# amisr/volumetricinterp

Measured on AMD Instinct MI355X. Metric: fit+eval timesteps/sec, higher is better.
Workload: dtype f64

## Files before the change

volumetricinterp_amd/csrc/vi_fit.hip:

```cpp
#include "vi_common.h"
#include "vi_solver.h"
#include "vi_gemm_device.h"

#include <rocsolver/rocsolver.h>

#include <cstdlib>

namespace {

inline unsigned nblk(int64_t n, int b) { return (unsigned)((n + b - 1) / b); }

__global__ void k_scale_rows(int64_t P, int N, const double* __restrict__ At, const double* __restrict__ W,
                             double* __restrict__ B, int tvalid)
{
    const int64_t p = (int64_t)blockIdx.x * blockDim.x + threadIdx.x;
    const int n = blockIdx.y, t = blockIdx.z;
    if (p >= P) return;
    const int ts = t < tvalid ? t : tvalid - 1;
    B[((int64_t)t * N + n) * P + p] = At[(int64_t)n * P + p] * W[(int64_t)ts * P + p];
}

__global__ void k_mul(int64_t n, const double* __restrict__ a, const double* __restrict__ b, double* __restrict__ o)
{
    const int64_t i = (int64_t)blockIdx.x * blockDim.x + threadIdx.x;
// ... 674 lines not shown
                                             tmp, N, s, d_H, N, s, &zero, d_dC, N, s, (rocblas_int)T));
    return VI_OK;
}

extern "C" int vi_eigvals_f64(vi_ctx* c, int64_t B, int32_t N, double* d_X, double* d_lam, int32_t* d_sweeps)
{
    VI_REQUIRE(c && d_X && d_lam, "null argument");
    VI_REQUIRE(B >= 0 && N > 0, "bad size");
    if (B == 0) return VI_OK;
    if (!vi_jacobi_supported(N)) {
        vi_set_error("vi_eigvals_f64: N=%d outside the in-LDS Jacobi range", N);
        return VI_ERR_UNSUPPORTED;
    }
    VI_HIP(hipSetDevice(c->device));
    const bool qr = qr_enabled(N);
    const size_t hhb = qr ? up16(vi_qr_hh_bytes(N)) : 0;
    cold_dst d{};
    d.cap = cold_max_sweeps(N);
    double* yz;
    int rc = ws_carve(c, [&](ws_carver& w) {
        d.log = w.take<char>((size_t)B * vi_jacobi_log_bytes(N, d.cap));
        d.scl = w.take<double>(B);
        yz = w.take<double>((size_t)B * N);
        d.C = w.take<double>((size_t)B * N);
        if (qr) {
            d.y1 = w.take<double>((size_t)B * N);
            d.hh = w.take<double>((size_t)B * (hhb / 8));
            d.scr = w.take<double>((size_t)B * N * N);
        }
    });
    if (rc != VI_OK) return rc;
    d.hh_stride = (int64_t)hhb;
    d.sweeps = d_sweeps;
    d.lam = d_lam;
    VI_HIP(hipMemsetAsync(yz, 0, (size_t)B * N * sizeof(double), c->stream));
    return cold_solve(c, B, N, d_X, yz, nullptr, 2.220446049250313e-16, d);
}

namespace {
size_t log_record_bytes(int N)
{
    return vi_jacobi_log_bytes(N, JACOBI_MAX_SWEEPS) + (qr_enabled(N) ? up16(vi_qr_hh_bytes(N)) : 0);
}

struct prep_ws {
    double *scl, *lam, *y1;
    double *T0, *T1;
    double *scrT, *scrD;
    const double** parr;
    int64_t np;
    void decompose(ws_carver& w, int64_t n, int N)
    {
        scl = w.take<double>(n);
        lam = w.take<double>((size_t)n * N);
        y1 = w.take<double>((size_t)n * N);
    }
    void matrices(ws_carver& w, int64_t n, int N)
    {
        T0 = w.take<double>((size_t)n * N * N);
        T1 = w.take<double>((size_t)n * N * N);
    }
    void finish(ws_carver& w, int64_t n, int N)
    {
        scrT = w.take<double>((size_t)GEMM_GROUP * N * N);
        scrD = w.take<double>((size_t)GEMM_GROUP * N * N);
        np = group_pad(n);
        parr = w.take<const double*>((size_t)6 * np);
    }
};

int prep_decompose(vi_ctx* c, int64_t bc, int N, const double* d_AWA, const int32_t* recc, const double* alpha0c,
                   const double* d_R, const double* d_y, double rcond, double* Cc, int32_t* rankc, void* log, int* nrd,
                   const prep_ws& p)
{
    hipLaunchKernelGGL(k_form_system, dim3((unsigned)bc), dim3(256), 0, c->stream, N * N, d_AWA, recc, alpha0c, d_R, p.T0);
    cold_dst d{};
    d.C = Cc;
    d.rank = rankc;
    d.C_back = true;
    d.log = log;
    d.hh = (double*)((char*)log + vi_jacobi_log_bytes(N, JACOBI_MAX_SWEEPS));
    d.log_stride = d.hh_stride = (int64_t)log_record_bytes(N);
    d.scl = p.scl;
    d.y1 = p.y1;
    d.scr = p.T1;
    d.lam = p.lam;
    d.lam_raw = 1;
    d.nround = nrd;
    d.cap = JACOBI_MAX_SWEEPS;
    return cold_solve(c, bc, N, p.T0, d_y, recc, rcond, d);
}

int prep_finish(vi_ctx* c, int64_t bc, int N, const void* log, const int* nrd, const double* d_AWA, const int32_t* recc,
                const double* d_R, const double* d_y, double* Vc, double* D1c, double* D2c, double* ytc, const prep_ws& p)
{
    const int NN = N * N;
    double *T0 = p.T0, *T1 = p.T1, *scrT = p.scrT, *scrD = p.scrD;
    const double** pT0 = p.parr;
    const double** pV = pT0 + p.np;
    const double** pT1 = pV + p.np;
    const double** pR = pT1 + p.np;
    const double** pD1 = pR + p.np;
    const double** pD2 = pD1 + p.np;
    const size_t recb = log_record_bytes(N);
    int rc = vi_jacobi_vectors(c, bc, N, log, JACOBI_MAX_SWEEPS, nrd, Vc, (int64_t)(recb / 16));
    if (rc != VI_OK) return rc;
    if (qr_enabled(N)) {
        const double* hh = (const double*)((const char*)log + vi_jacobi_log_bytes(N, JACOBI_MAX_SWEEPS));
        if ((rc = vi_qr_back_mat(c, bc, N, hh, Vc, (int64_t)(recb / 8))) != VI_OK) return rc;
    }
    hipLaunchKernelGGL(k_form_system, dim3((unsigned)bc), dim3(256), 0, c->stream, NN, d_AWA, recc, nullptr, nullptr, T0);
    VI_HIP(hipGetLastError());
    if ((rc = group_ptrs(c, bc, T0, NN, nullptr, 0, pT0)) != VI_OK) return rc;
    if ((rc = group_ptrs(c, bc, Vc, NN, nullptr, 0, pV)) != VI_OK) return rc;
    if ((rc = group_ptrs(c, bc, T1, NN, scrT, NN, pT1)) != VI_OK) return rc;
    if ((rc = group_ptrs(c, bc, d_R, 0, nullptr, 0, pR)) != VI_OK) return rc;
    if ((rc = group_ptrs(c, bc, D1c, NN, scrD, NN, pD1)) != VI_OK) return rc;
    if ((rc = group_ptrs(c, bc, D2c, NN, scrD, NN, pD2)) != VI_OK) return rc;
    if ((rc = gemm_groups(c, rocblas_operation_none, rocblas_operation_none, N, N, N, pT0, N, pV, N, pT1, N, bc)) != VI_OK) return rc;
    if ((rc = gemm_groups(c, rocblas_operation_transpose, rocblas_operation_none, N, N, N, pV, N, pT1, N, pD1, N, bc)) != VI_OK)
        return rc;
    if ((rc = gemm_groups(c, rocblas_operation_none, rocblas_operation_none, N, N, N, pR, N, pV, N, pT1, N, bc)) != VI_OK) return rc;
    if ((rc = gemm_groups(c, rocblas_operation_transpose, rocblas_operation_none, N, N, N, pV, N, pT1, N, pD2, N, bc)) != VI_OK)
        return rc;
    hipLaunchKernelGGL(k_vt_vec, dim3((unsigned)bc), dim3(256), 0, c->stream, N, Vc, nullptr, d_y, recc, ytc);
    VI_HIP(hipGetLastError());
    return VI_OK;
}
}

extern "C" int vi_warm_prepare_f64(vi_ctx* c, int64_t B, int32_t N, const double* d_AWA, const int32_t* d_rec,
                                   const double* d_alpha0, const double* d_R, const double* d_y, double rcond,
                                   double* d_C, int32_t* d_rank, double* d_V, double* d_D1, double* d_D2, double* d_yt)
{
    VI_REQUIRE(c && d_AWA && d_rec && d_alpha0 && d_R && d_y && d_C && d_V && d_D1 && d_D2 && d_yt, "null argument");
    VI_REQUIRE(B >= 0 && N > 0, "bad size");
    if (B == 0) return VI_OK;
    if (!vi_jacobi_vectors_supported(N)) {
        vi_set_error("vi_warm_prepare_f64: N=%d outside the in-LDS Jacobi range", N);
        return VI_ERR_UNSUPPORTED;
    }
    VI_HIP(hipSetDevice(c->device));
    const int NN = N * N;
    const size_t recb = log_record_bytes(N);
    const size_t per = recb + (size_t)(2 * N + 1) * sizeof(double) + sizeof(int) + (size_t)2 * NN * sizeof(double) + 6 * sizeof(void*);
    const int64_t Bc = chunk_size((size_t)4 << 30, per, B);
    void* log;
    int* nrd;
    prep_ws p{};
    int rc = ws_carve(c, [&](ws_carver& w) {
        log = w.take<char>((size_t)Bc * recb);
        p.decompose(w, Bc, N);
        p.matrices(w, Bc, N);
        p.finish(w, Bc, N);
        nrd = w.take<int>(Bc);
    });
    if (rc != VI_OK) return rc;
    return for_chunks(B, Bc, [&](int64_t i0, int64_t bc) -> int {
        const int r = prep_decompose(c, bc, N, d_AWA, d_rec + i0, d_alpha0 + i0, d_R, d_y, rcond, d_C + i0 * N,
                                     d_rank ? d_rank + i0 : nullptr, log, nrd, p);
        if (r != VI_OK) return r;
        return prep_finish(c, bc, N, log, nrd, d_AWA, d_rec + i0, d_R, d_y, d_V + i0 * NN, d_D1 + i0 * NN, d_D2 + i0 * NN,
                           d_yt + i0 * N, p);
    });
}

extern "C" size_t vi_rotation_log_bytes(int32_t N) { return log_record_bytes(N); }
extern "C" int vi_max_sweeps(void) { return JACOBI_MAX_SWEEPS; }
extern "C" int vi_cold_max_sweeps(int32_t N) { return cold_max_sweeps(N); }
double vi_floor_warm() { return JACOBI_FLOOR_WARM; }

namespace {
double walk_tolerance()
{
    static const double v = vi_env_double("VINTERP_WALK_TOL", 1e-6);
    return v;
}
}

extern "C" int vi_decompose_f64(vi_ctx* c, int64_t B, int32_t N, const double* d_AWA, const int32_t* d_rec,
                                const double* d_alpha0, const double* d_R, const double* d_y, double rcond, double* d_C,
                                int32_t* d_rank, void* d_log, int32_t* d_nround)
{
    VI_REQUIRE(c && d_AWA && d_rec && d_alpha0 && d_R && d_y && d_C && d_log && d_nround, "null argument");
    VI_REQUIRE(B >= 0 && N > 0, "bad size");
    if (B == 0) return VI_OK;
    if (!vi_jacobi_vectors_supported(N)) {
        vi_set_error("vi_decompose_f64: N=%d outside the in-LDS Jacobi range", N);
        return VI_ERR_UNSUPPORTED;
    }
    VI_HIP(hipSetDevice(c->device));
    prep_ws p{};
    int rc = ws_carve(c, [&](ws_carver& w) {
        p.decompose(w, B, N);
        p.matrices(w, B, N);
    });
    if (rc != VI_OK) return rc;
    return prep_decompose(c, B, N, d_AWA, d_rec, d_alpha0, d_R, d_y, rcond, d_C, d_rank, d_log, d_nround, p);
}

extern "C" int vi_warm_finish_f64(vi_ctx* c, int64_t B, int32_t N, const void* d_log, const int32_t* d_nround,
                                  const double* d_AWA, const int32_t* d_rec, const double* d_R, const double* d_y,
                                  double* d_V, double* d_D1, double* d_D2, double* d_yt)
{
    VI_REQUIRE(c && d_log && d_nround && d_AWA && d_rec && d_R && d_y && d_V && d_D1 && d_D2 && d_yt, "null argument");
    VI_REQUIRE(B >= 0 && N > 0, "bad size");
    if (B == 0) return VI_OK;
    if (!vi_jacobi_vectors_supported(N)) {
        vi_set_error("vi_warm_finish_f64: N=%d outside the in-LDS Jacobi range", N);
        return VI_ERR_UNSUPPORTED;
    }
    VI_HIP(hipSetDevice(c->device));
    prep_ws p{};
    int rc = ws_carve(c, [&](ws_carver& w) {
        p.matrices(w, B, N);
        p.finish(w, B, N);
    });
    if (rc != VI_OK) return rc;
    return prep_finish(c, B, N, d_log, d_nround, d_AWA, d_rec, d_R, d_y, d_V, d_D1, d_D2, d_yt, p);
}

extern "C" int vi_warm_solve_f64(vi_ctx* c, int64_t B, int32_t N, const double* d_D1, const double* d_D2,
                                 const double* d_yt, const double* d_V, const int32_t* d_slot, const double* d_alpha,
                                 double rcond, double* d_C, int32_t* d_rank, int32_t* d_sweeps)
{
    VI_REQUIRE(c && d_D1 && d_D2 && d_yt && d_V && d_slot && d_alpha && d_C, "null argument");
    VI_REQUIRE(B >= 0 && N > 0, "bad size");
    if (B == 0) return VI_OK;
    if (!vi_jacobi_supported(N)) {
        vi_set_error("vi_warm_solve_f64: N=%d outside the in-LDS Jacobi range", N);
        return VI_ERR_UNSUPPORTED;
    }
    VI_HIP(hipSetDevice(c->device));
    const int NN = N * N;
    const size_t logb = vi_jacobi_log_bytes(N, JACOBI_MAX_SWEEPS);
    const int64_t Bc = chunk_size((size_t)4 << 30, logb, B);
    void* log;
    double *scl, *X, *cp;
    int rc = ws_carve(c, [&](ws_carver& w) {
        log = w.take<char>((size_t)Bc * logb);
        scl = w.take<double>(Bc);
        X = w.take<double>((size_t)Bc * NN);
        cp = w.take<double>((size_t)Bc * N);
    });
    if (rc != VI_OK) return rc;
    return for_chunks(B, Bc, [&](int64_t i0, int64_t bc) -> int {
        form_pair_scaled(c, bc, NN, d_D1, d_D2, d_slot + i0, d_slot + i0, d_alpha + i0, X, scl);
        VI_HIP(hipGetLastError());
        const int r = vi_jacobi_solve(c, bc, N, X, scl, d_yt, d_slot + i0, rcond, cp, d_rank ? d_rank + i0 : nullptr, log,
                                      JACOBI_MAX_SWEEPS, d_sweeps ? d_sweeps + i0 : nullptr, nullptr, 0, nullptr, JACOBI_FLOOR_WARM);
        if (r != VI_OK) return r;
        hipLaunchKernelGGL(k_v_vec, dim3((unsigned)bc), dim3(256), (size_t)N * sizeof(double), c->stream, N, d_V,
                           d_slot + i0, cp, d_C + i0 * N);
        VI_HIP(hipGetLastError());
        return VI_OK;
    });
}

namespace {
template <int BS>
__global__ __launch_bounds__(BS) void k_reg_floor(int NN, const double* __restrict__ AWA, const double* __restrict__ R,
                                                  double* __restrict__ out)
{
    __shared__ double red[BS / 64];
    const double* Xt = AWA + (int64_t)blockIdx.x * NN;
    double mn = 1.7976931348623157e308;
    for (int e = threadIdx.x; e < NN; e += BS) {
        const double r = fabs(R[e]);
        if (r > 0.0) mn = fmin(mn, (0.25 * 2.220446049250313e-16) * fabs(Xt[e]) / r);
    }
    for (int o = 32; o > 0; o >>= 1) mn = fmin(mn, __shfl_xor(mn, o));
    if ((threadIdx.x & 63) == 0) red[threadIdx.x >> 6] = mn;
    __syncthreads();
    if (threadIdx.x == 0) {
        for (int q = 1; q < BS / 64; ++q) mn = fmin(mn, red[q]);
        out[blockIdx.x] = mn;
    }
}
}

extern "C" int vi_reg_floor_f64(vi_ctx* c, int64_t T, int32_t N, const double* d_AWA, const double* d_R, double* d_out)
{
    VI_REQUIRE(c && d_AWA && d_R && d_out, "null argument");
    VI_REQUIRE(T >= 0 && N > 0, "bad size");
    if (T == 0) return VI_OK;
    VI_HIP(hipSetDevice(c->device));
    hipLaunchKernelGGL(k_reg_floor<256>, dim3((unsigned)T), dim3(256), 0, c->stream, N * N, d_AWA, d_R, d_out);
    VI_HIP(hipGetLastError());
    return VI_OK;
}

namespace {
__global__ void k_basis_ptrs(int64_t B, int NN, const double* AWA, const int* __restrict__ rec, const double* V,
                             const int* __restrict__ basis, double* T1, double* D1, const double** pA, const double** pV,
                             double** pT, double** pD)
{
    const int64_t i = (int64_t)blockIdx.x * blockDim.x + threadIdx.x;
    if (i >= B) return;
    pA[i] = AWA + (int64_t)rec[i] * NN;
    pV[i] = V + (int64_t)basis[i] * NN;
    pT[i] = T1 + i * NN;
    pD[i] = D1 + i * NN;
}
}

extern "C" int vi_basis_solve_f64(vi_ctx* c, int64_t B, int32_t N, const double* d_AWA, const double* d_y,
                                  const int32_t* d_rec, const int32_t* d_basis, const double* d_alpha, const double* d_V,
                                  const double* d_D2, double rcond, double* d_C, int32_t* d_rank, int32_t* d_sweeps)
{
    VI_REQUIRE(c && d_AWA && d_y && d_rec && d_basis && d_alpha && d_V && d_D2 && d_C, "null argument");
    VI_REQUIRE(B >= 0 && N > 0, "bad size");
    if (B == 0) return VI_OK;
    if (!vi_jacobi_supported(N)) {
        vi_set_error("vi_basis_solve_f64: N=%d outside the in-LDS Jacobi range", N);
        return VI_ERR_UNSUPPORTED;
    }
    VI_HIP(hipSetDevice(c->device));
    const int NN = N * N;
    const size_t logb = vi_jacobi_log_bytes(N, JACOBI_MAX_SWEEPS);
    const size_t per = logb + sizeof(double) + (size_t)2 * NN * sizeof(double) + (size_t)2 * N * sizeof(double) + 4 * sizeof(void*);
    const int64_t Bc = chunk_size((size_t)8 << 30, per, B, 256);
    void* log;
    double *scl, *T1, *D1, *yt, *cp;
    const double **pA, **pV;
    double **pT, **pD;
    int rc = ws_carve(c, [&](ws_carver& w) {
        log = w.take<char>((size_t)Bc * logb);
        scl = w.take<double>(Bc);
        T1 = w.take<double>((size_t)Bc * NN);
        D1 = w.take<double>((size_t)Bc * NN);
        yt = w.take<double>((size_t)Bc * N);
        cp = w.take<double>((size_t)Bc * N);
        pA = w.take<const double*>(Bc);
        pV = w.take<const double*>(Bc);
        pT = w.take<double*>(Bc);
        pD = w.take<double*>(Bc);
    });
    if (rc != VI_OK) return rc;
    const double one = 1.0, zero = 0.0;
    return for_chunks(B, Bc, [&](int64_t i0, int64_t bc) -> int {
        hipLaunchKernelGGL(k_basis_ptrs, dim3((unsigned)((bc + 255) / 256)), dim3(256), 0, c->stream, bc, NN, d_AWA,
                           d_rec + i0, d_V, d_basis + i0, T1, D1, pA, pV, pT, pD);
        VI_HIP(hipGetLastError());
        VI_ROCBLAS(rocblas_dgemm_batched(c->blas, rocblas_operation_none, rocblas_operation_none, N, N, N, &one, pA, N,
                                         pV, N, &zero, pT, N, (rocblas_int)bc));
        VI_ROCBLAS(rocblas_dgemm_batched(c->blas, rocblas_operation_transpose, rocblas_operation_none, N, N, N, &one, pV, N,
                                         (const double* const*)pT, N, &zero, pD, N, (rocblas_int)bc));
        hipLaunchKernelGGL(k_vt_vec, dim3((unsigned)bc), dim3(256), 0, c->stream, N, d_V, d_basis + i0, d_y, d_rec + i0, yt);
        form_pair_scaled(c, bc, NN, D1, d_D2, nullptr, d_basis + i0, d_alpha + i0, D1, scl);
        VI_HIP(hipGetLastError());
        const int r = vi_jacobi_solve(c, bc, N, D1, scl, yt, nullptr, rcond, cp, d_rank ? d_rank + i0 : nullptr, log,
                                      JACOBI_MAX_SWEEPS, d_sweeps ? d_sweeps + i0 : nullptr, nullptr, 0, nullptr,
                                      JACOBI_FLOOR_WARM, 0, walk_tolerance());
        if (r != VI_OK) return r;
        hipLaunchKernelGGL(k_v_vec, dim3((unsigned)bc), dim3(256), (size_t)N * sizeof(double), c->stream, N, d_V,
                           d_basis + i0, cp, d_C + i0 * N);
        VI_HIP(hipGetLastError());
        return VI_OK;
    });
}

extern "C" int vi_warm_rebase_f64(vi_ctx* c, int64_t B, int64_t nplain, int32_t N, const double* d_AWA, const double* d_R,
                                  const double* d_y, const int32_t* d_rec, const int32_t* d_slot, const double* d_alpha,
                                  double rcond, double* d_V, double* d_D1, double* d_D2, double* d_yt, double* d_C,
                                  int32_t* d_rank, int32_t* d_sweeps)
{
    VI_REQUIRE(c && d_AWA && d_R && d_y && d_rec && d_slot && d_alpha && d_V && d_D1 && d_D2 && d_yt && d_C, "null argument");
    VI_REQUIRE(B >= 0 && N > 0 && nplain >= 0 && nplain <= B, "bad size");
    if (B == 0) return VI_OK;
    if (nplain == B) return vi_warm_solve_f64(c, B, N, d_D1, d_D2, d_yt, d_V, d_slot, d_alpha, rcond, d_C, d_rank, d_sweeps);
    if (!vi_jacobi_vectors_supported(N)) {
        vi_set_error("vi_warm_rebase_f64: N=%d outside the in-LDS Jacobi range", N);
        return VI_ERR_UNSUPPORTED;
    }
    VI_HIP(hipSetDevice(c->device));
    const int NN = N * N;
    const size_t logb = vi_jacobi_log_bytes(N, JACOBI_MAX_SWEEPS);
    const size_t per = logb + sizeof(double) + sizeof(int) + (size_t)3 * NN * sizeof(double) + (size_t)N * sizeof(double) +
                       8 * sizeof(void*);
    const int64_t Bc = chunk_size((size_t)4 << 30, per, B);
    if (nplain > 0 && B > Bc) {
        int rc0 = vi_warm_solve_f64(c, nplain, N, d_D1, d_D2, d_yt, d_V, d_slot, d_alpha, rcond, d_C, d_rank, d_sweeps);
        if (rc0 != VI_OK) return rc0;
        return vi_warm_rebase_f64(c, B - nplain, 0, N, d_AWA, d_R, d_y, d_rec + nplain, d_slot + nplain, d_alpha + nplain, rcond,
                                  d_V, d_D1, d_D2, d_yt, d_C + nplain * N, d_rank ? d_rank + nplain : nullptr,
                                  d_sweeps ? d_sweeps + nplain : nullptr);
    }
    const int64_t Bcp = group_pad(Bc);
    char* log;
    double *scl, *X, *Vw, *Vn, *cp, *scrA, *scrB;
    const double **pX, **pVold, **pVw, **pVn, **pR, **pD1, **pD2;
    int* nrd;
    int rc = ws_carve(c, [&](ws_carver& w) {
        log = w.take<char>((size_t)Bc * logb);
        scl = w.take<double>(Bc);
        X = w.take<double>((size_t)Bc * NN);
        Vw = w.take<double>((size_t)Bc * NN);
        Vn = w.take<double>((size_t)Bc * NN);
        cp = w.take<double>((size_t)Bc * N);
        scrA = w.take<double>((size_t)GEMM_GROUP * NN);
        scrB = w.take<double>((size_t)GEMM_GROUP * NN);
        for (auto* pp : {&pX, &pVold, &pVw, &pVn, &pR, &pD1, &pD2}) *pp = w.take<const double*>(Bcp);
        nrd = w.take<int>(Bc);
    });
    if (rc != VI_OK) return rc;
    return for_chunks(B, Bc, [&](int64_t i0, int64_t bc) -> int {
        const int32_t* slotc = d_slot + i0;
        const int32_t* recc = d_rec + i0;
        form_pair_scaled(c, bc, NN, d_D1, d_D2, slotc, slotc, d_alpha + i0, X, scl);
        VI_HIP(hipGetLastError());
        int rc = vi_jacobi_solve(c, bc, N, X, scl, d_yt, slotc, rcond, cp, d_rank ? d_rank + i0 : nullptr, log, JACOBI_MAX_SWEEPS,
                                 d_sweeps ? d_sweeps + i0 : nullptr, nullptr, 0, nrd, JACOBI_FLOOR_WARM);
        if (rc != VI_OK) return rc;
        hipLaunchKernelGGL(k_v_vec, dim3((unsigned)bc), dim3(256), (size_t)N * sizeof(double), c->stream, N, d_V, slotc, cp,
                           d_C + i0 * N);
        VI_HIP(hipGetLastError());
        const int64_t skip = i0 == 0 ? nplain : 0;
        rc = vi_jacobi_vectors(c, bc - skip, N, log + (size_t)skip * logb, JACOBI_MAX_SWEEPS, nrd + skip, Vw);
        if (rc != VI_OK) return rc;
        slotc += skip;
        recc += skip;
        bc -= skip;
        if ((rc = group_ptrs(c, bc, d_V, NN, nullptr, 0, pVold, slotc)) != VI_OK) return rc;
        if ((rc = group_ptrs(c, bc, Vw, NN, scrA, NN, pVw)) != VI_OK) return rc;
        if ((rc = group_ptrs(c, bc, Vn, NN, scrB, NN, pVn)) != VI_OK) return rc;
        if ((rc = wg_gemm_batched(c, false, N, pVold, pVw, pVn, bc)) != VI_OK) return rc;
        hipLaunchKernelGGL(k_scatter_mat, dim3((unsigned)bc), dim3(256), 0, c->stream, NN, Vn, slotc, d_V);
        hipLaunchKernelGGL(k_form_system, dim3((unsigned)bc), dim3(256), 0, c->stream, NN, d_AWA, recc, nullptr, nullptr, X);
        VI_HIP(hipGetLastError());
        if ((rc = group_ptrs(c, bc, X, NN, nullptr, 0, pX)) != VI_OK) return rc;
        if ((rc = group_ptrs(c, bc, d_R, 0, nullptr, 0, pR)) != VI_OK) return rc;
        if ((rc = group_ptrs(c, bc, d_D1, NN, scrB, NN, pD1, slotc)) != VI_OK) return rc;
        if ((rc = group_ptrs(c, bc, d_D2, NN, scrB, NN, pD2, slotc)) != VI_OK) return rc;
        if ((rc = wg_gemm_batched(c, false, N, pX, pVn, pVw, bc)) != VI_OK) return rc;
        if ((rc = wg_gemm_batched(c, true, N, pVn, pVw, pD1, bc)) != VI_OK) return rc;
        if ((rc = wg_gemm_batched(c, false, N, pR, pVn, pVw, bc)) != VI_OK) return rc;
        if ((rc = wg_gemm_batched(c, true, N, pVn, pVw, pD2, bc)) != VI_OK) return rc;
        hipLaunchKernelGGL(k_vt_vec_slot, dim3((unsigned)bc), dim3(256), 0, c->stream, N, Vn, d_y, recc, slotc, d_yt);
        VI_HIP(hipGetLastError());
        return VI_OK;
    });
}

namespace {
__global__ void k_set_one(double* scratch, double alpha, int slot, int rec)
{
    scratch[0] = alpha;
    int* iv = reinterpret_cast<int*>(scratch + 2);
    iv[0] = slot;
    iv[1] = rec;
}
}

extern "C" int vi_warm_chi2_one_f64(vi_ctx* c, int32_t N, int64_t P, const double* d_D1, const double* d_D2,
                                    const double* d_yt, const double* d_V, int32_t slot, double alpha, double rcond,
                                    const double* d_At, int32_t rec, const double* d_W, const double* d_b,
                                    double* d_scratch, double* h_chi2)
{
    VI_REQUIRE(c && d_D1 && d_D2 && d_yt && d_V && d_At && d_W && d_b && d_scratch && h_chi2, "null argument");
    VI_REQUIRE(N > 0 && P > 0 && slot >= 0 && rec >= 0, "bad size");
    VI_HIP(hipSetDevice(c->device));
    double* d_alpha = d_scratch;
    double* d_chi = d_scratch + 1;
    int32_t* d_slot = reinterpret_cast<int32_t*>(d_scratch + 2);
    int32_t* d_rec = d_slot + 1;
    int32_t* d_sw = reinterpret_cast<int32_t*>(d_scratch + 3);
    double* d_C = d_scratch + 8;
    hipLaunchKernelGGL(k_set_one, dim3(1), dim3(1), 0, c->stream, d_scratch, alpha, (int)slot, (int)rec);
    VI_HIP(hipGetLastError());
    int rc = vi_warm_solve_f64(c, 1, N, d_D1, d_D2, d_yt, d_V, d_slot, d_alpha, rcond, d_C, nullptr, d_sw);
    if (rc != VI_OK) return rc;
    rc = vi_chi2_f64(c, 1, P, N, d_At, d_C, d_rec, d_W, d_b, d_chi);
    if (rc != VI_OK) return rc;
    VI_HIP(hipMemcpyAsync(h_chi2, d_chi, 3 * sizeof(double), hipMemcpyDeviceToHost, c->stream));
    VI_HIP(hipStreamSynchronize(c->stream));
    return VI_OK;
}

extern "C" int vi_gcv_terms_f64(vi_ctx* c, int64_t np, int64_t P, int32_t N, const double* d_At, const int32_t* d_pidx,
                                const double* d_AWA, const double* d_y, const double* d_W, const double* d_b,
                                double alpha, const double* d_R, double rcond, double* d_res)
{
    VI_REQUIRE(c && d_At && d_pidx && d_AWA && d_y && d_W && d_b && d_res, "null argument");
    VI_REQUIRE(np >= 0 && P > 0 && N > 0, "bad size");
    if (np == 0) return VI_OK;
    VI_HIP(hipSetDevice(c->device));
    const int NN = N * N;
    const int64_t Bc = chunk_size((size_t)1 << 30, (size_t)NN * sizeof(double), np);
    double* buf = nullptr;
    VI_HIP(hipMalloc((void**)&buf, (size_t)Bc * (NN + 2 * (size_t)N) * sizeof(double)));
    double* X = buf;
    double* yl = X + (size_t)Bc * NN;
    double* Cl = yl + (size_t)Bc * N;
    const int rc = for_chunks(np, Bc, [&](int64_t i0, int64_t bc) -> int {
        hipLaunchKernelGGL(k_form_loo, dim3((unsigned)bc), dim3(256), (size_t)N * sizeof(double), c->stream, N, P, d_At,
                           d_pidx + i0, d_AWA, d_y, d_W, d_b, alpha, d_R, X, yl);
        if (hipGetLastError() != hipSuccess) { vi_set_error("k_form_loo launch failed"); return VI_ERR_HIP; }
        const int r = vi_solve_trunc_f64(c, bc, N, X, yl, nullptr, rcond, Cl, nullptr, 0.0, nullptr);
        if (r != VI_OK) return r;
        hipLaunchKernelGGL(k_loo_resid, dim3((unsigned)((bc + 3) / 4)), dim3(256), 0, c->stream, bc, N, P, d_At, d_pidx + i0,
                           Cl, d_W, d_b, d_res + i0);
        if (hipGetLastError() != hipSuccess) { vi_set_error("k_loo_resid launch failed"); return VI_ERR_HIP; }
        return VI_OK;
    });
    (void)hipStreamSynchronize(c->stream);
    (void)hipFree(buf);
    return rc;
}
```

volumetricinterp_amd/csrc/vi_solver.h:

```cpp
#pragma once
#include "vi_common.h"

size_t vi_jacobi_lds_bytes(int N);
size_t vi_jacobi_log_bytes(int N, int max_sweeps);
bool vi_jacobi_supported(int N);
bool vi_jacobi_use_v2(int N);
int vi_jacobi_solve(vi_ctx* c, int64_t B, int N, const double* d_X, const double* d_scl, const double* d_y,
                    const int* d_rec, double rcond, double* d_C, int* d_rank, void* d_log, int max_sweeps,
                    int* d_sweeps, double* d_lam, int lam_raw, int* d_nround, double abs_floor, int64_t log_stride = 0,
                    double conv_tol = 0.0);
bool vi_jacobi_vectors_supported(int N);
int vi_jacobi_vectors(vi_ctx* c, int64_t B, int N, const void* d_log, int max_sweeps, const int* d_nround, double* d_V,
                      int64_t log_stride = 0);

bool vi_qr_supported(int N);
size_t vi_qr_hh_bytes(int N);
int vi_qr_precond(vi_ctx* c, int64_t B, int N, const double* d_X, const double* d_y, const int* d_rec, double* d_X1,
                  double* d_y1, double* d_hh, double* d_scr, int64_t hh_stride = 0);
int vi_qr_back_vec(vi_ctx* c, int64_t B, int N, const double* d_hh, double* d_C, int64_t hh_stride = 0);
int vi_qr_back_mat(vi_ctx* c, int64_t B, int N, const double* d_hh, double* d_V, int64_t hh_stride = 0);

double vi_floor_warm();

int vi_eval_sph_mfma(vi_model* m, int64_t Q, const double* lat, const double* lon, const double* alt, int64_t T,
                     const double* Cp, const unsigned char* hull, int F, double* out, int64_t* done);
int vi_eval_sph_split(vi_model* m, int64_t Q, const double* lat, const double* lon, const double* alt, int64_t T,
                      const double* Cp, const unsigned char* hull, int F, double* out, int* handled);
int vi_eval_resident_mfma(vi_ctx* c, int N, int64_t Q, int64_t T, const double* d_Y, const double* d_C, double* d_out, int* handled);
int vi_eval_resident_err_mfma(vi_ctx* c, int N, int64_t Q, int64_t T, const double* d_Y, const double* d_dC, double* d_out,
                              int* handled);
```

Measured before the change: 3365.

## Fuse basis rotation V^T A V, projection and scaling into one MFMA kernel

Replaces the two batched rocBLAS DGEMMs, the pointer-setup kernel, the V^T y kernel and the pair-scaling pass in the basis solve with one per-item kernel. The new kernel computes V^T·A·V with f64 MFMA, keeps V and A in registers or LDS, writes only the lower-triangular blocks, adds alpha·D2, and applies a power-of-two scale. This removes several launches and the global round trip of the intermediate T1 matrix, and halves the workspace per item, which allows larger chunks. The old BLAS path stays available through an environment variable. The risks are that each block handles one matrix, which may leave the GPU underused for small N, and that the non-resident path for large N reloads V from global memory.

After: 3435, median of 6. +2.1%, better.

```diff
diff --git a/volumetricinterp_amd/csrc/vi_fit.hip b/volumetricinterp_amd/csrc/vi_fit.hip
--- a/volumetricinterp_amd/csrc/vi_fit.hip
+++ b/volumetricinterp_amd/csrc/vi_fit.hip
@@ -1000,6 +1000,17 @@
     pT[i] = T1 + i * NN;
     pD[i] = D1 + i * NN;
 }
+
+bool walk_form_blas()
+{
+    static const bool v = vi_env_is("VINTERP_WALK_FORM", "blas");
+    return v;
+}
+int walk_chunk_cap()
+{
+    static const int v = vi_env_int("VINTERP_WALK_CHUNK", 0);
+    return v;
+}
 }
 
 extern "C" int vi_basis_solve_f64(vi_ctx* c, int64_t B, int32_t N, const double* d_AWA, const double* d_y,
@@ -1015,39 +1026,49 @@
     }
     VI_HIP(hipSetDevice(c->device));
     const int NN = N * N;
+    const bool blas = walk_form_blas();
     const size_t logb = vi_jacobi_log_bytes(N, JACOBI_MAX_SWEEPS);
-    const size_t per = logb + sizeof(double) + (size_t)2 * NN * sizeof(double) + (size_t)2 * N * sizeof(double) + 4 * sizeof(void*);
-    const int64_t Bc = chunk_size((size_t)8 << 30, per, B, 256);
+    size_t per = logb + sizeof(double) + (size_t)NN * sizeof(double) + (size_t)2 * N * sizeof(double);
+    if (blas) per += (size_t)NN * sizeof(double) + 4 * sizeof(void*);
+    int64_t Bc = chunk_size((size_t)8 << 30, per, B, 256);
+    if (walk_chunk_cap() > 0 && Bc > walk_chunk_cap()) Bc = walk_chunk_cap();
     void* log;
-    double *scl, *T1, *D1, *yt, *cp;
-    const double **pA, **pV;
-    double **pT, **pD;
+    double *scl, *T1 = nullptr, *X, *yt, *cp;
+    const double **pA = nullptr, **pV = nullptr;
+    double **pT = nullptr, **pD = nullptr;
     int rc = ws_carve(c, [&](ws_carver& w) {
         log = w.take<char>((size_t)Bc * logb);
         scl = w.take<double>(Bc);
-        T1 = w.take<double>((size_t)Bc * NN);
-        D1 = w.take<double>((size_t)Bc * NN);
+        X = w.take<double>((size_t)Bc * NN);
         yt = w.take<double>((size_t)Bc * N);
         cp = w.take<double>((size_t)Bc * N);
-        pA = w.take<const double*>(Bc);
-        pV = w.take<const double*>(Bc);
-        pT = w.take<double*>(Bc);
-        pD = w.take<double*>(Bc);
+        if (blas) {
+            T1 = w.take<double>((size_t)Bc * NN);
+            pA = w.take<const double*>(Bc);
+            pV = w.take<const double*>(Bc);
+            pT = w.take<double*>(Bc);
+            pD = w.take<double*>(Bc);
+        }
     });
     if (rc != VI_OK) return rc;
     const double one = 1.0, zero = 0.0;
     return for_chunks(B, Bc, [&](int64_t i0, int64_t bc) -> int {
-        hipLaunchKernelGGL(k_basis_ptrs, dim3((unsigned)((bc + 255) / 256)), dim3(256), 0, c->stream, bc, NN, d_AWA,
-                           d_rec + i0, d_V, d_basis + i0, T1, D1, pA, pV, pT, pD);
-        VI_HIP(hipGetLastError());
-        VI_ROCBLAS(rocblas_dgemm_batched(c->blas, rocblas_operation_none, rocblas_operation_none, N, N, N, &one, pA, N,
-                                         pV, N, &zero, pT, N, (rocblas_int)bc));
-        VI_ROCBLAS(rocblas_dgemm_batched(c->blas, rocblas_operation_transpose, rocblas_operation_none, N, N, N, &one, pV, N,
-                                         (const double* const*)pT, N, &zero, pD, N, (rocblas_int)bc));
-        hipLaunchKernelGGL(k_vt_vec, dim3((unsigned)bc), dim3(256), 0, c->stream, N, d_V, d_basis + i0, d_y, d_rec + i0, yt);
-        form_pair_scaled(c, bc, NN, D1, d_D2, nullptr, d_basis + i0, d_alpha + i0, D1, scl);
-        VI_HIP(hipGetLastError());
-        const int r = vi_jacobi_solve(c, bc, N, D1, scl, yt, nullptr, rcond, cp, d_rank ? d_rank + i0 : nullptr, log,
+        if (blas) {
+            hipLaunchKernelGGL(k_basis_ptrs, dim3((unsigned)((bc + 255) / 256)), dim3(256), 0, c->stream, bc, NN, d_AWA,
+                               d_rec + i0, d_V, d_basis + i0, T1, X, pA, pV, pT, pD);
+            VI_HIP(hipGetLastError());
+            VI_ROCBLAS(rocblas_dgemm_batched(c->blas, rocblas_operation_none, rocblas_operation_none, N, N, N, &one, pA, N,
+                                             pV, N, &zero, pT, N, (rocblas_int)bc));
+            VI_ROCBLAS(rocblas_dgemm_batched(c->blas, rocblas_operation_transpose, rocblas_operation_none, N, N, N, &one, pV,
+                                             N, (const double* const*)pT, N, &zero, pD, N, (rocblas_int)bc));
+            hipLaunchKernelGGL(k_vt_vec, dim3((unsigned)bc), dim3(256), 0, c->stream, N, d_V, d_basis + i0, d_y, d_rec + i0, yt);
+            form_pair_scaled(c, bc, NN, X, d_D2, nullptr, d_basis + i0, d_alpha + i0, X, scl);
+            VI_HIP(hipGetLastError());
+        } else {
+            const int r = vi_walk_rotate(c, bc, N, d_AWA, d_rec + i0, d_V, d_D2, d_basis + i0, d_y, d_alpha + i0, X, scl, yt);
+            if (r != VI_OK) return r;
+        }
+        const int r = vi_jacobi_solve(c, bc, N, X, scl, yt, nullptr, rcond, cp, d_rank ? d_rank + i0 : nullptr, log,
                                       JACOBI_MAX_SWEEPS, d_sweeps ? d_sweeps + i0 : nullptr, nullptr, 0, nullptr,
                                       JACOBI_FLOOR_WARM, 0, walk_tolerance());
         if (r != VI_OK) return r;
diff --git a/volumetricinterp_amd/csrc/vi_solver.h b/volumetricinterp_amd/csrc/vi_solver.h
--- a/volumetricinterp_amd/csrc/vi_solver.h
+++ b/volumetricinterp_amd/csrc/vi_solver.h
@@ -20,6 +20,9 @@
 int vi_qr_back_vec(vi_ctx* c, int64_t B, int N, const double* d_hh, double* d_C, int64_t hh_stride = 0);
 int vi_qr_back_mat(vi_ctx* c, int64_t B, int N, const double* d_hh, double* d_V, int64_t hh_stride = 0);
 
+int vi_walk_rotate(vi_ctx* c, int64_t B, int N, const double* d_AWA, const int* d_rec, const double* d_V, const double* d_D2,
+                   const int* d_basis, const double* d_y, const double* d_alpha, double* d_X, double* d_scl, double* d_yt);
+
 double vi_floor_warm();
 
 int vi_eval_sph_mfma(vi_model* m, int64_t Q, const double* lat, const double* lon, const double* alt, int64_t T,
diff --git a/volumetricinterp_amd/csrc/vi_walk.hip b/volumetricinterp_amd/csrc/vi_walk.hip
--- /dev/null
+++ b/volumetricinterp_amd/csrc/vi_walk.hip
@@ -0,0 +1,200 @@
+#include "vi_common.h"
+#include "vi_solver.h"
+
+namespace {
+
+using v4f64 = __attribute__((__vector_size__(4 * sizeof(double)))) double;
+
+template <int NT, bool RES, int KL, bool PAD>
+__global__ __launch_bounds__(NT * 64) void k_walk_rotate(int N, const double* __restrict__ AWA, const int* __restrict__ rec,
+                                                         const double* __restrict__ V, const double* __restrict__ D2,
+                                                         const int* __restrict__ basis, const double* __restrict__ y,
+                                                         const double* __restrict__ alpha, double* __restrict__ X,
+                                                         double* __restrict__ scl, double* __restrict__ yt)
+{
+    constexpr int KS = 4 * NT;
+    constexpr int UNR = RES ? NT : 1;
+    __shared__ double shV[KS * 64];
+    __shared__ double shW[KS * 64];
+    __shared__ double shB[KL > 0 ? NT * KL * 64 : 1];
+    __shared__ double red[NT];
+    const int64_t i = blockIdx.x;
+    const int tid = threadIdx.x, lane = tid & 63, w = tid >> 6;
+    const int n = lane & 15, g = lane >> 4;
+    const int64_t NN = (int64_t)N * N;
+    const double* Ai = AWA + (int64_t)rec[i] * NN;
+    const double* Vi = V + (int64_t)basis[i] * NN;
+    const double* D2i = D2 + (int64_t)basis[i] * NN;
+    const double* yi = y + (int64_t)rec[i] * N;
+    double* Xi = X + i * NN;
+    const double a = alpha[i];
+    const int c = 16 * w + n;
+    const bool cok = c < N;
+
+    const int cc = (!PAD || cok) ? c : N - 1;
+    auto loadA = [&](int u) {
+        const int k = 4 * u + g;
+        if (!PAD) return Ai[(int64_t)k * N + c];
+        return Ai[(int64_t)(k < N ? k : N - 1) * N + cc] * ((cok && k < N) ? 1.0 : 0.0);
+    };
+    auto loadV = [&](int blk, int u) {
+        const int r = 16 * blk + n, k = 4 * u + g;
+        if (!PAD) return Vi[(int64_t)r * N + k];
+        return Vi[(int64_t)(r < N ? r : N - 1) * N + (k < N ? k : N - 1)] * ((r < N && k < N) ? 1.0 : 0.0);
+    };
+    for (int k = w; k < N; k += NT) {
+        double acc = 0.0;
+        for (int r = lane; r < N; r += 64) acc = fma(Vi[(int64_t)k * N + r], yi[r], acc);
+        for (int o = 32; o > 0; o >>= 1) acc += __shfl_down(acc, o);
+        if (lane == 0) yt[i * N + k] = acc;
+    }
+
+    constexpr int KR = KS - KL;
+    double bA[RES ? KS : 1], bV[RES ? KR : 1];
+    if (RES) {
+#pragma unroll
+        for (int u = 0; u < KS; ++u) bA[u] = loadA(u);
+#pragma unroll
+        for (int u = 0; u < KR; ++u) bV[u] = loadV(w, u);
+#pragma unroll
+        for (int u = KR; u < KS; ++u) shB[(w * KL + u - KR) * 64 + lane] = loadV(w, u);
+    }
+    auto getV = [&](int u) { return !RES ? loadV(w, u) : u < KR ? bV[u] : shB[(w * KL + u - KR) * 64 + lane]; };
+
+    double mx = 0.0;
+    for (int I = 0; I < NT; ++I) {
+        if (RES) {
+            if (w == I) {
+#pragma unroll
+                for (int u = 0; u < KS; ++u) shV[u * 64 + lane] = getV(u);
+            }
+        } else {
+            for (int u = w; u < KS; u += NT) shV[u * 64 + lane] = loadV(I, u);
+        }
+        __syncthreads();
+        v4f64 t = {0.0, 0.0, 0.0, 0.0};
+#pragma unroll UNR
+        for (int u0 = 0; u0 < KS; u0 += 4) {
+            double av[4];
+#pragma unroll
+            for (int u = 0; u < 4; ++u) av[u] = shV[(u0 + u) * 64 + lane];
+#pragma unroll
+            for (int u = 0; u < 4; ++u)
+                t = __builtin_amdgcn_mfma_f64_16x16x4f64(av[u], RES ? bA[u0 + u] : loadA(u0 + u), t, 0, 0, 0);
+            __builtin_amdgcn_sched_barrier(0);
+        }
+#pragma unroll
+        for (int r = 0; r < 4; ++r) shW[(4 * w + (n >> 2)) * 64 + (g + 4 * r) + 16 * (n & 3)] = t[r];
+        __syncthreads();
+        if (w <= I) {
+            double d2v[4];
+#pragma unroll
+            for (int r = 0; r < 4; ++r) {
+                const int row = 16 * I + g + 4 * r;
+                d2v[r] = (!PAD || (cok && row < N)) ? D2i[(int64_t)row * N + c] : 0.0;
+            }
+            v4f64 d = {0.0, 0.0, 0.0, 0.0};
+#pragma unroll UNR
+            for (int u0 = 0; u0 < KS; u0 += 4) {
+                double av[4];
+#pragma unroll
+                for (int u = 0; u < 4; ++u) av[u] = shW[(u0 + u) * 64 + lane];
+#pragma unroll
+                for (int u = 0; u < 4; ++u)
+                    d = __builtin_amdgcn_mfma_f64_16x16x4f64(av[u], getV(u0 + u), d, 0, 0, 0);
+                __builtin_amdgcn_sched_barrier(0);
+            }
+#pragma unroll
+            for (int r = 0; r < 4; ++r) {
+                const int row = 16 * I + g + 4 * r;
+                if (!PAD || (cok && row < N)) {
+                    const double v = fma(a, d2v[r], d[r]);
+                    mx = fmax(mx, fabs(v));
+                    Xi[(int64_t)row * N + c] = v;
+                }
+            }
+        }
+    }
+
+    for (int o = 32; o > 0; o >>= 1) mx = fmax(mx, __shfl_xor(mx, o));
+    if (lane == 0) red[w] = mx;
+    __syncthreads();
+    mx = 0.0;
+#pragma unroll
+    for (int q = 0; q < NT; ++q) mx = fmax(mx, red[q]);
+    int ex = 0;
+    double f = 1.0;
+    if (mx > 0.0 && mx < 1.7e308) {
+        (void)frexp(mx, &ex);
+        f = ldexp(1.0, 1 - ex);
+    }
+    constexpr int RB = 8, CG = (16 * NT + 63) / 64;
+    for (int r0 = w; r0 < N; r0 += RB * NT) {
+        double xv[RB][CG];
+#pragma unroll
+        for (int q = 0; q < RB; ++q) {
+            const int row = r0 + q * NT < N ? r0 + q * NT : N - 1;
+            const int lim = 16 * (row / 16 + 1) < N ? 16 * (row / 16 + 1) : N;
+#pragma unroll
+            for (int m = 0; m < CG; ++m) {
+                const int col = lane + 64 * m;
+                xv[q][m] = Xi[(int64_t)row * N + (col < lim ? col : lim - 1)];
+            }
+        }
+#pragma unroll
+        for (int q = 0; q < RB; ++q) {
+            const int row = r0 + q * NT;
+            const int lim = 16 * (row / 16 + 1) < N ? 16 * (row / 16 + 1) : N;
+#pragma unroll
+            for (int m = 0; m < CG; ++m) {
+                const int col = lane + 64 * m;
+                if (row < N && col < lim) Xi[(int64_t)row * N + col] = xv[q][m] * f;
+            }
+        }
+    }
+    if (tid == 0) scl[i] = 1.0 / f;
+}
+
+template <int NT, bool RES, int KL, bool RESP>
+void launch_walk_rotate(vi_ctx* c, int64_t B, int N, const double* AWA, const int* rec, const double* V, const double* D2,
+                        const int* basis, const double* y, const double* alpha, double* X, double* scl, double* yt)
+{
+    if (N == 16 * NT)
+        hipLaunchKernelGGL((k_walk_rotate<NT, RES, KL, false>), dim3((unsigned)B), dim3(NT * 64), 0, c->stream, N, AWA, rec, V, D2,
+                           basis, y, alpha, X, scl, yt);
+    else
+        hipLaunchKernelGGL((k_walk_rotate<NT, RESP, 0, true>), dim3((unsigned)B), dim3(NT * 64), 0, c->stream, N, AWA, rec, V, D2,
+                           basis, y, alpha, X, scl, yt);
+}
+
+}
+
+int vi_walk_rotate(vi_ctx* c, int64_t B, int N, const double* d_AWA, const int* d_rec, const double* d_V, const double* d_D2,
+                   const int* d_basis, const double* d_y, const double* d_alpha, double* d_X, double* d_scl, double* d_yt)
+{
+#define VI_W(NT, RES, KL, RESP)                                                                                                \
+    case NT:                                                                                                          \
+        launch_walk_rotate<NT, RES, KL, RESP>(c, B, N, d_AWA, d_rec, d_V, d_D2, d_basis, d_y, d_alpha, d_X, d_scl, d_yt);       \
+        break
+    switch ((N + 15) / 16) {
+        VI_W(1, true, 0, true);
+        VI_W(2, true, 0, true);
+        VI_W(3, true, 0, true);
+        VI_W(4, true, 0, true);
+        VI_W(5, true, 0, true);
+        VI_W(6, true, 0, true);
+        VI_W(7, true, 0, true);
+        VI_W(8, true, 0, true);
+        VI_W(9, true, 16, false);
+        VI_W(10, false, 0, false);
+        VI_W(11, false, 0, false);
+        VI_W(12, false, 0, false);
+        VI_W(13, false, 0, false);
+    default:
+        vi_set_error("vi_walk_rotate: N=%d outside 1..208", N);
+        return VI_ERR_UNSUPPORTED;
+    }
+#undef VI_W
+    VI_HIP(hipGetLastError());
+    return VI_OK;
+}
```
